# zepfu/llama-gguf-inference

Measured on AMD Instinct MI355X. Metric: decode tokens/sec + achieved HBM GB/s, Llama-3-8B Q4_K_M, 1->8 MI355X, higher is better.
Workload: dtype int8; 1 GPU; llama3-8b-q4km: 128-token prompt -> greedy decode on the 128->640 trajectory, 1521 timed tokens at positions 133..1653 (mean context of the trajectory), 1 replica per GPU; model=llama3-8b-q4km, parallelism=replicas x1 (RCCL weight fan-out), global_batch=1

## Files before the change

### llama-gguf-inference_amd/csrc/capi_hooks.cpp

```cpp
#include <hip/hip_runtime.h>

#include <algorithm>
#include <cstring>
#include <string>
#include <vector>

#include "../../include/llmi.h"
#include "capi_internal.h"

using namespace llmi;

extern "C" {

int32_t llmi_profile_kernels(struct llama_context* ctx, llama_token first, int32_t pos0, int32_t n_steps, double* us,
                             double* bytes, int32_t* launches) {
    API_TRY
    if (!ctx || n_steps <= 0 || !us || !bytes || !launches) { set_err("llmi_profile_kernels: bad arguments"); return -1; }
    Context& c = ctx->c;
    if (first < 0 || first >= c.m->hp.n_vocab || pos0 < 0 || pos0 >= c.n_ctx) {
        set_err("llmi_profile_kernels: token/position out of range");
        return -1;
    }
    (void)hipSetDevice(c.m->device);
    const int kv_bound = std::min(c.n_ctx, (pos0 / 256 + 1) * 256);
// ... 54 lines not shown
    if (!c.le_trace && hipMalloc(&c.le_trace, n * 8) != hipSuccess) { set_err("llmi_engine_trace: hipMalloc"); return -3; }
    (void)hipMemsetAsync(c.le_trace, 0, n * 8, c.stream);
    bool ok = launch_state_set(c.st, first, pos0, c.stream) == hipSuccess && step_enqueue(c, kv_bound, err);
    c.le_trace_layer = layer;
    ok = ok && launch_state_set(c.st, first, pos0, c.stream) == hipSuccess && step_enqueue(c, kv_bound, err);
    c.le_trace_layer = -1;
    if (!ok || hipMemcpyAsync(out, c.le_trace, n * 8, hipMemcpyDeviceToHost, c.stream) != hipSuccess ||
        hipStreamSynchronize(c.stream) != hipSuccess) {
        set_err("llmi_engine_trace: " + (err.empty() ? std::string("launch failed") : err));
        rc = -4;
    }
    if (launch_state_set(c.st, first, pos0, c.stream) != hipSuccess || hipStreamSynchronize(c.stream) != hipSuccess)
        if (rc == 0) { set_err("llmi_engine_trace: state reset failed"); rc = -4; }
    c.n_past = pos0;
    return rc == 0 ? cus : rc;
    API_CATCH(-5)
}

double llmi_le_stream_bench(const void* src, int64_t bytes, int32_t mode, int32_t iters, int32_t nt) {
    return le_stream_bench(src, (size_t)bytes, mode, iters, nt);
}

static thread_local int t_hook_numerics = 0;

int32_t llmi_test_option(const char* name, int32_t value) {
    if (!name) return -1;
    int* opt = nullptr;
    if (!strcmp(name, "numerics")) {
        const int old = t_hook_numerics;
        if (value >= 0 && value <= (NUMERICS_X86 | NUMERICS_FA)) t_hook_numerics = value;
        else if (value >= 0) { set_err("llmi_test_option: numerics must be 0..3"); return -1; }
        return old;
    }
    if (!strcmp(name, "pf_attn_simple")) opt = &g_pf_attn_simple;
    else if (!strcmp(name, "pf_fa_noalloc")) opt = &g_pf_fa_noalloc;
    else if (!strcmp(name, "pf_attn_fa")) opt = &g_pf_attn_fa;
    else if (!strcmp(name, "pf_gemm_ng")) opt = &g_pf_gemm_ng;
    else if (!strcmp(name, "pf_qkv_merge")) opt = &g_pf_qkv_merge;
    else if (!strcmp(name, "pf_xcd_map")) opt = &g_pf_xcd_map;
    else if (!strcmp(name, "pf_quant_bpc")) opt = &g_pf_quant_bpc;
    else if (!strcmp(name, "pf_quant_split_below")) opt = &g_pf_quant_split_below;
    else if (!strcmp(name, "pf_fa_cfg")) opt = &g_pf_fa_cfg;
    else if (!strcmp(name, "pf_max_kv")) opt = &g_pf_max_kv;
    else if (!strcmp(name, "xspin_limit")) opt = &g_xspin_limit;
    else if (!strcmp(name, "xtag_skew")) opt = &g_xtag_skew;
    else if (!strcmp(name, "engine")) opt = &g_le_on;
    else if (!strcmp(name, "le_spin")) opt = &g_le_spin;
    if (!opt) { set_err("llmi_test_option: unknown option"); return -1; }
    const int old = *opt;
    if (value >= 0) *opt = value;
    return old;
}

int32_t llmi_debug_tap(struct llama_context* ctx, int32_t which, float* out) {
    if (!ctx || !out) { set_err("llmi_debug_tap: bad arguments"); return -1; }
    Context& c = ctx->c;
    const HParams& hp = c.m->hp;
    (void)hipSetDevice(c.m->device);
    if (which == 7 || which == 8) {
        const size_t kvl = (size_t)hp.n_head_kv * c.n_ctx * hp.head_dim;
        const uint16_t* base = (which == 7 ? c.kc : c.vc) + (size_t)(hp.n_layer - 1) * kvl;
        hipError_t e = hipMemcpyAsync(out, base, kvl * 2, hipMemcpyDeviceToHost, c.stream);
        if (e == hipSuccess) e = hipStreamSynchronize(c.stream);
        if (e != hipSuccess) { set_err(hip_err(e)); return -2; }
        return 0;
    }
    if (which >= 11 && which <= 15) {
// ... 600 lines not shown
```

### llama-gguf-inference_amd/csrc/kernels.h

```cpp
#pragma once

#include <hip/hip_runtime.h>

#include <cstdint>
#include <string>

#include "common.h"

namespace llmi {

#ifndef LLMI_MV_THREADS
#define LLMI_MV_THREADS 256
#endif
constexpr int kMVThreads = LLMI_MV_THREADS;
constexpr int kMVWaves = kMVThreads / 64;
constexpr int kFusedAttnMaxKV = 8192;
constexpr size_t kSplitAttnMaxLds = 128 * 1024;
constexpr int kXAttnMaxKV = 1024;
constexpr int kDimAttnMaxKV = 1024;
constexpr int kRegAttnMaxKV = 512;
constexpr int kPfAttnMaxKV = 32768;
extern int g_pf_fa_noalloc, g_pf_gemm_ng, g_pf_qkv_merge, g_pf_xcd_map, g_pf_quant_bpc, g_pf_quant_split_below, g_pf_attn_simple, g_pf_attn_fa, g_pf_fa_cfg, g_pf_max_kv, g_xspin_limit, g_xtag_skew;
int pf_max_kv();
__host__ __device__ inline size_t attn_gran_off(int n_head, int n_ctx) {
    return ((size_t)n_head * n_ctx + (size_t)n_head * (n_ctx / 32 + 1) + 3) & ~(size_t)3;
}
constexpr int kLongTile = 256;
__host__ __device__ inline size_t attn_long_off(int n_head, int n_ctx) { return attn_gran_off(n_head, n_ctx) + 2 * (size_t)n_head * kXAttnMaxKV + 4; }
inline size_t attn_scratch_floats(int n_head, int n_ctx) {
    return attn_long_off(n_head, n_ctx) + 2 * (size_t)n_head * ((n_ctx + kLongTile - 1) / kLongTile) * 129;
}

enum Epi : int { EPI_STORE = 0, EPI_ADD = 1, EPI_QKV = 2, EPI_SWIGLU = 3, EPI_LOGITS = 4,
                 EPI_SWIGLU_UP = 5 };

struct Seg {
    const uint8_t* a = nullptr;
    const uint8_t* h = nullptr;
    const uint8_t* s = nullptr;
    const uint8_t* d = nullptr;
    int type = -1;
    int rows = 0;
    int row0 = 0;
    int rgs = 0;
    int x86 = 0;
};

struct MVArgs {
    Seg seg[3];
    int nseg = 0;
    int cols = 0;
    int npairs = 0;
    const float* x = nullptr;
    const float* nw = nullptr;
    const uint8_t* xq = nullptr;
    float eps = 0.f;
    float* y = nullptr;
    uint16_t* kc = nullptr;
    uint16_t* vc = nullptr;
    const float* rope = nullptr;
    StepState* st = nullptr;
    int head_dim = 0, n_rot = 0, n_ctx = 0, nq = 0, nk = 0;
    unsigned long long* argmax = nullptr;
    unsigned long long* trace = nullptr;
    int lr = 0;
    int rpt = 0;
    int ntasks = 0;
    int split_tasks = 0;
    int split_wgs = 0;
    int xfirst = 0;
    int fw = 0;
    int prio_alt = 0;
    int x_stride = 0, y_stride = 0;
    const int* tpos = nullptr;
    const int* tseq = nullptr;
    size_t kv_stride = 0;
    int num = 0;
};

constexpr int kLeOps = 4;
struct LeArgs {
    MVArgs op[kLeOps];
    int nops = 0;
    unsigned* cnt = nullptr;
    size_t cnt_stride = 0;
    unsigned* fault = nullptr;
    int spin_limit = 0;
    int kmin = 9;
    int npieces = 0, img_off0 = 0, img_off1 = 0, fold_off = 0, ring_off = 0, act = -1;
    int exp = 0;
    unsigned long long* trace = nullptr;
};
size_t le_counter_bytes(int n_layer);
size_t le_counter_stride(int n_layer);
hipError_t layer_engine_prepare(LeArgs& a);
hipError_t launch_layer_engine(const LeArgs& a, hipStream_t s);
double le_stream_bench(const void* src, size_t bytes, int mode, int iters, int nt);
bool le_wanted();
extern int g_le_on, g_le_spin;

// ... 70 lines not shown
    const float* rope = nullptr;
    int pos0 = 0, head_dim = 0, n_rot = 0, n_ctx = 0;
    int exp = 0;
};
struct PfAttn {
    const float* q = nullptr;
    float* out = nullptr;
    int ldq = 0;
    const uint16_t* kc = nullptr, *vc = nullptr;
    int n_ctx = 0, pos0 = 0, gqa = 1, max_kv = 0;
    float scale = 0.f;
    float* wsc = nullptr;
    size_t wsc_bytes = 0;
    int num = 0;
    int fa = 0;
};
size_t pf_fa_scratch_bytes(int n_head, int n_head_kv, int head_dim, int T, int n_ctx);
constexpr size_t kPfFaScratchCap = (size_t)1 << 30;
bool pf_gemm_ok(int type, int rows, int cols);
hipError_t launch_pf_embed(const Seg& w, int cols, int vocab, const int32_t* toks, float* X, int T, int32_t* hist,
                           int pos0, int n_ctx, hipStream_t s);
hipError_t launch_pf_quant(const float* x, int ldx, const float* nw, float eps, int cols, int act, int T, void* aq,
                           int16_t* abs, float* ad, void* abf, hipStream_t s, int x86 = 0);
hipError_t launch_pf_gemm(const PfGemm& g, int epi, hipStream_t s);
hipError_t launch_pf_attn(const PfAttn& a, int n_head, int head_dim, int T, hipStream_t s, int path = -1);

__host__ __device__ inline int act_kind(int t) { return t == T_Q8_0 ? 1 : 0; }
bool mv_geometry(MVArgs& a, int epi);
size_t mv_lds_bytes(int act, int cols);
template <int ACT, bool NORM, int T, int X86>
hipError_t mv_dispatch_epi(const MVArgs& a, int epi, dim3 grid, size_t lds, hipStream_t s);
template <bool NORM, int T, int T2, int X86>
hipError_t mv_qkv2_launch(const MVArgs& a, int split_tasks, dim3 grid, size_t lds, hipStream_t s);

hipError_t launch_matvec(const MVArgs& a, int epi, int max_blocks, hipStream_t stream);
int attn_path(int n_head, int n_head_kv, int kv_bound, int head_dim, int mode = -1);
int attn_d_slices(int n_head, int head_dim);
int battn_path(int g, int n_head, int head_dim, int kv_bound, int nt);
int battn_slices(int n_head, int head_dim, int kv_bound, int nt);
int attn_passes(int kv_bound, int cap);
struct LongGeo { int ntile, np, nscores; };
LongGeo attn_long_geo(int kv_bound);
void set_launch_events(hipEvent_t start, hipEvent_t stop);
void set_attn_mode(int mode);
constexpr int kFaMaxKV = 8192;
hipError_t launch_attention_fa(const AttnArgs& a, int n_head, int n_head_kv, int head_dim, int kv_bound, hipStream_t s);
hipError_t launch_battention_fa(const BAttnArgs& b, int nt, int n_head, int n_head_kv, int head_dim, int kv_bound,
                                hipStream_t s);
hipError_t launch_battention_x86(const BAttnArgs& b, int nt, int n_head, int n_head_kv, int head_dim, int kv_bound,
                                 hipStream_t s);
hipError_t launch_attention(const AttnArgs& a, int n_head, int n_head_kv, int head_dim, int kv_bound, hipStream_t stream,
                            int mode = -1);
hipError_t launch_embed(const EmbArgs& a, hipStream_t stream);
hipError_t launch_embed_row(const EmbArgs& a, const StepState* st, float* out, hipStream_t stream);
hipError_t launch_repack(int type, const void* raw, uint8_t* a, uint8_t* h, uint8_t* s, uint8_t* d, int64_t nblk, int64_t cols, int rgs,
                         int x86, hipStream_t stream);
hipError_t launch_attention_x86(const AttnArgs& a, int n_head, int n_head_kv, int head_dim, int kv_bound, hipStream_t s,
                                int mode = 0);
hipError_t launch_pf_attn_x86(const PfAttn& a, int n_head, int n_head_kv, int head_dim, int T, hipStream_t s);
int pf_attn_x86_max_kv(int n_head, int n_head_kv, int head_dim);
hipError_t launch_pf_attn_fa(const PfAttn& a, int n_head, int head_dim, int T, hipStream_t s);
hipError_t launch_quant_dump(const MVArgs& a, int act, void* out, hipStream_t stream);
hipError_t launch_stream_read(const void* p, size_t bytes, unsigned* out, int blocks, hipStream_t stream);
hipError_t launch_arena_hash(const void* p, size_t bytes, unsigned long long* out, hipStream_t stream);
hipError_t launch_state_set(StepState* st, int token_in, int pos_next, hipStream_t stream);
hipError_t launch_state_tick(StepState* st, hipStream_t stream);
// ... 3 lines not shown
```

### llama-gguf-inference_amd/csrc/kernels.hip

```cpp
#include "kernels.h"
#include "mv_device.h"
#include "launch_util.h"

#include <algorithm>
#include <cstdlib>

#include <hip/hip_runtime.h>

namespace llmi {

static thread_local hipEvent_t t_ev_start = nullptr, t_ev_stop = nullptr;
void set_launch_events(hipEvent_t start, hipEvent_t stop) {
    t_ev_start = start;
    t_ev_stop = stop;
}
hipEvent_t launch_event(bool stop) { return stop ? t_ev_stop : t_ev_start; }

size_t mv_lds_bytes(int act, int cols) { return fold_off(act, cols, kMVWaves) + (size_t)kMVWaves * kFoldFloats * 4; }

template <int ACT, int X86>
__global__ __launch_bounds__(kMVThreads) void k_quant_dump(MVArgs A, uint8_t* out) {
    extern __shared__ __attribute__((aligned(16))) uint8_t smem[];
    const Lds L = carve(smem, ACT, A.cols);
    if (A.nw) mv_prologue<ACT, true, X86>(A, L);
    else mv_prologue<ACT, false, X86>(A, L);
    __syncthreads();
    const int cols = A.cols;
    for (int e = threadIdx.x; e < cols; e += blockDim.x) {
        const uint8_t* rec = L.act + (size_t)(e >> 8) * kRec;
        const int t = e & 255;
        if (ACT == 0) {
            const int c = t >> 6, h = (t >> 5) & 1, l = X86 ? (t & 31) >> 2 : t & 7, i = X86 ? t & 3 : (t & 31) >> 3;
            out[(size_t)(e >> 8) * 292 + 4 + t] = rec[32 * (2 * c + (l >> 2)) + 16 * h + 4 * (l & 3) + i];
        } else {
            out[(size_t)(e >> 5) * 34 + 2 + (e & 31)] = rec[t];
        }
    }
    if (ACT == 0) {
// ... 198 lines not shown
    const int sp = split_row / a.rpt;
#define LLMI_QKV2(A_, B_)                                                                            \
    if (t1 == A_ && t2 == B_) return mv_qkv2_launch<NORM, A_, B_, X86>(a, sp, grid, lds, s);
    if constexpr (NORM) {
        LLMI_QKV2(T_Q4_K, T_Q6_K) LLMI_QKV2(T_Q4_K, T_Q5_K) LLMI_QKV2(T_Q5_K, T_Q6_K)
    }
#undef LLMI_QKV2
    return hipErrorNotSupported;
}

template <bool NORM, int X86>
static hipError_t mv_dispatch_type(const MVArgs& a, int epi, dim3 grid, size_t lds, hipStream_t s) {
    static const bool qkv2 = !getenv("LLMI_NO_QKV2");
    if (epi == EPI_QKV && qkv2) {
        const hipError_t e = mv_dispatch_qkv2<NORM, X86>(a, grid, lds, s);
        if (e != hipErrorNotSupported) return e;
    }
    int best = a.seg[0].type, best_rows = 0;
    for (int i = 0; i < a.nseg; ++i) {
        int rows = 0;
        for (int k = 0; k < a.nseg; ++k)
            if (a.seg[k].type == a.seg[i].type) rows += a.seg[k].rows;
        if (rows > best_rows) { best_rows = rows; best = a.seg[i].type; }
    }
    switch (best) {
        case T_Q4_K: return mv_dispatch_epi<0, NORM, T_Q4_K, X86>(a, epi, grid, lds, s);
        case T_Q5_K: return mv_dispatch_epi<0, NORM, T_Q5_K, X86>(a, epi, grid, lds, s);
        case T_Q6_K: return mv_dispatch_epi<0, NORM, T_Q6_K, X86>(a, epi, grid, lds, s);
        case T_Q8_0: return mv_dispatch_epi<1, NORM, T_Q8_0, X86>(a, epi, grid, lds, s);
        default: return hipErrorInvalidValue;
    }
}

bool mv_geometry(MVArgs& a, int epi) {
    if (a.nseg < 1 || a.cols < 256 || a.cols % 256) return false;
    const int U = a.cols >> 8, lmax = epi == EPI_QKV ? 32 : 64;
    static const int lr_cap = [] {
        const char* e = getenv("LLMI_MV_LR");
        return e ? atoi(e) : 64;
    }();
    int lr = (std::min(std::min(U, lmax), lr_cap) + 3) & ~3;
    lr = std::min(std::max(lr, 4), lmax);
    int R = 1;
    while (2 * R * lr <= 64) R *= 2;
    auto aligned = [&](int r) {
        for (int i = 1; i < a.nseg; ++i)
            if ((a.seg[i].row0 - a.seg[0].row0) % r) return false;
        return true;
    };
    if (epi != EPI_SWIGLU)
        while (R > 1 && !aligned(R)) R >>= 1;
    if (epi == EPI_QKV && R < 2) return false;
    int rows;
    if (epi == EPI_SWIGLU) {
        if (a.nseg != 2 || a.seg[0].rows != a.seg[1].rows) return false;
        rows = a.seg[0].rows;
    } else {
        rows = a.seg[a.nseg - 1].row0 + a.seg[a.nseg - 1].rows - a.seg[0].row0;
    }
    a.lr = lr;
    a.rpt = R;
    a.ntasks = (rows + R - 1) / R;
    return a.ntasks > 0;
}

static int mv_fw() {
    static const int v = [] {
        const char* e = getenv("LLMI_MV_FW");
        return e ? atoi(e) : 0;
    }();
    return v;
}

hipError_t launch_matvec(const MVArgs& a0, int epi, int max_blocks, hipStream_t s) {
    if (a0.nseg < 1 || a0.cols <= 0 || a0.cols % 256) return hipErrorInvalidValue;
    MVArgs a = a0;
    a.fw = mv_fw();
    if (!mv_geometry(a, epi)) return hipErrorInvalidValue;
    const int act = act_kind(a.seg[0].type);
    for (int i = 1; i < a.nseg; ++i)
        if (act_kind(a.seg[i].type) != act) return hipErrorInvalidValue;
    const size_t lds = mv_lds_bytes(act, a.cols);
    if (lds > 160 * 1024) return hipErrorInvalidValue;
    int blocks = (a.ntasks + kMVWaves - 1) / kMVWaves;
    if (blocks > max_blocks) blocks = max_blocks;
#if defined(LLMI_EXPERIMENTS)
    static const int exp_blocks = [] {
        const char* e = getenv("LLMI_MV_BLOCKS");
        return e ? atoi(e) : 0;
    }();
    if (exp_blocks > 0 && exp_blocks < blocks) blocks = exp_blocks;
#endif
    const dim3 grid(blocks);
    for (int i = 0; i < a.nseg; ++i)
        if ((a.seg[i].x86 != 0) != (a.num != 0)) return hipErrorInvalidValue;
    if (a.num) return a.nw ? mv_dispatch_type<true, 1>(a, epi, grid, lds, s) : mv_dispatch_type<false, 1>(a, epi, grid, lds, s);
    return a.nw ? mv_dispatch_type<true, 0>(a, epi, grid, lds, s) : mv_dispatch_type<false, 0>(a, epi, grid, lds, s);
}

hipError_t launch_quant_dump(const MVArgs& a, int act, void* out, hipStream_t s) {
    if (a.cols <= 0 || a.cols % 256) return hipErrorInvalidValue;
    const size_t lds = mv_lds_bytes(act, a.cols);
    if (a.num) {
        if (act == 0) hipLaunchKernelGGL((k_quant_dump<0, 1>), dim3(1), dim3(kMVThreads), lds, s, a, (uint8_t*)out);
        else hipLaunchKernelGGL((k_quant_dump<1, 1>), dim3(1), dim3(kMVThreads), lds, s, a, (uint8_t*)out);
    } else {
        if (act == 0) hipLaunchKernelGGL((k_quant_dump<0, 0>), dim3(1), dim3(kMVThreads), lds, s, a, (uint8_t*)out);
        else hipLaunchKernelGGL((k_quant_dump<1, 0>), dim3(1), dim3(kMVThreads), lds, s, a, (uint8_t*)out);
    }
    return hipGetLastError();
}
// ... 48 lines not shown
```

### llama-gguf-inference_amd/csrc/mv_device.h

```cpp
#pragma once

#include <hip/hip_runtime.h>

#include "kernels.h"
#include "../../include/llmi_math.h"

namespace llmi {

typedef unsigned int u32x4 __attribute__((ext_vector_type(4)));
typedef unsigned int u32x2 __attribute__((ext_vector_type(2)));
typedef int i32x4 __attribute__((ext_vector_type(4)));
typedef short short2_t __attribute__((ext_vector_type(2)));

#ifndef LLMI_NT
#define LLMI_NT 1
#endif
constexpr bool kNontemporalWeights = LLMI_NT != 0;

__device__ __forceinline__ float h2f(uint32_t h) {
    return (float)__builtin_bit_cast(_Float16, (uint16_t)(h & 0xffffu));
}
__device__ __forceinline__ uint16_t f2h(float f) {
    __asm__("" : "+v"(f));
    return __builtin_bit_cast(uint16_t, (_Float16)f);
// ... 1072 lines not shown
__device__ __forceinline__ void task_any(const MA& A, const Lds& L, float* F, const TaskGeo& g, int task, int r, int ul,
                                         int pos, unsigned long long& best) {
    const int S = EPI == EPI_SWIGLU ? 2 * g.nj : g.nj;
    float acc = 0.f, vg = 0.f;
    for (int s = 0; s < S; ++s) {
        const Sub b = sub_of<EPI>(A, g, task, s);
        const Seg sg = pick(A, b.si);
        const LaneUnit lu = lane_unit(g, b, sg, r, ul);
        const uint8_t* rec = L.act + (size_t)lu.u * kRec;
        float tm[9];
        if constexpr (X86) {
            if constexpr (ACT == 1) {
                unit_store_x86<T_Q8_0>(load_unit<T_Q8_0>(sg, lu.row, lu.u, g.U), rec, F, r, ul, g.lr, g.R, lu.valid);
            } else {
                switch (sg.type) {
                    case T_Q4_K: unit_store_x86<T_Q4_K>(load_unit<T_Q4_K>(sg, lu.row, lu.u, g.U), rec, F, r, ul, g.lr, g.R, lu.valid); break;
                    case T_Q5_K: unit_store_x86<T_Q5_K>(load_unit<T_Q5_K>(sg, lu.row, lu.u, g.U), rec, F, r, ul, g.lr, g.R, lu.valid); break;
                    default: unit_store_x86<T_Q6_K>(load_unit<T_Q6_K>(sg, lu.row, lu.u, g.U), rec, F, r, ul, g.lr, g.R, lu.valid); break;
                }
            }
        } else if constexpr (ACT == 1) {
            unit_terms<T_Q8_0>(load_unit<T_Q8_0>(sg, lu.row, lu.u, g.U), rec, tm);
        } else {
            switch (sg.type) {
                case T_Q4_K: unit_terms<T_Q4_K>(load_unit<T_Q4_K>(sg, lu.row, lu.u, g.U), rec, tm); break;
                case T_Q5_K: unit_terms<T_Q5_K>(load_unit<T_Q5_K>(sg, lu.row, lu.u, g.U), rec, tm); break;
                default: unit_terms<T_Q6_K>(load_unit<T_Q6_K>(sg, lu.row, lu.u, g.U), rec, tm); break;
            }
        }
        sub_finish<ACT, EPI, MA, X86>(A, F, g, s, b, sg, tm, lu, r, ul, acc, vg, pos, best);
    }
}

__device__ __forceinline__ float dequant_elem(const Seg& w, int row, int e, int cols) {
    const size_t U = (size_t)(cols >> 8), u = (size_t)(e >> 8), ru = (size_t)row * U + u;
    switch (w.type) {
        case T_F32: return ((const float*)w.a)[(size_t)row * cols + e];
        case T_F16: return h2f(((const uint16_t*)w.a)[(size_t)row * cols + e]);
        case T_Q4_K:
        case T_Q5_K:
        case T_Q6_K: {
            const int t = e & 255, c = t >> 6, hi = (t >> 5) & 1;
            const int l = w.x86 ? (t & 31) >> 2 : t & 7, i = w.x86 ? t & 3 : (t & 31) >> 3, k = l >> 2, m = l & 3;
            const uint8_t qb = w.a[piece_off(row, 2 * c + k, u, U, 8, w.rgs) + 4 * m + i];
            int q = hi ? (qb >> 4) : (qb & 0xF);
            if (w.type == T_Q6_K) {
                const uint8_t hb = w.h[piece_off(row, c, u, U, 4, w.rgs) + (2 * hi + k) * 4 + i];
                q |= (((hb >> (2 * m)) & 3) ^ 2) << 4;
                const float d = h2f(*(const uint16_t*)(w.d + ru * 2));
                const int sc = (int8_t)w.s[ru * 16 + (t >> 4)];
                return d * (float)sc * (float)(q - 32);
            }
            const uint32_t* s32 = (const uint32_t*)(w.s + ru * 16);
            int sc, mn;
            scale_min(2 * c + hi, s32[1], s32[2], s32[3], sc, mn);
            if (w.type == T_Q5_K) {
                const uint8_t hb = w.h[piece_off(row, c >> 1, u, U, 2, w.rgs) + 8 * (c & 1) + 4 * hi + i];
                q += ((hb >> l) & 1) << 4;
            }
            const float d = h2f(s32[0]), dmin = h2f(s32[0] >> 16);
            const float d1 = d * (float)sc, m1 = dmin * (float)mn;
            return d1 * (float)q - m1;
        }
        case T_Q8_0: {
            const int t = e & 255;
            const uint8_t qb = w.a[piece_off(row, t >> 4, u, U, 16, w.rgs) + (t & 15)];
// ... 20 lines not shown
```

### llama-gguf-inference_amd/csrc/mv_kernels.h

```cpp
#pragma once
#include "kernels.h"
#include "launch_util.h"
#include "mv_device.h"

#include <algorithm>
#include <cstdlib>
#include <map>
#include <mutex>
#include <tuple>

namespace llmi {

#ifndef LLMI_MV_PINGPONG
#define LLMI_MV_PINGPONG 1
#endif
#ifndef LLMI_Q6_MASKED
#define LLMI_Q6_MASKED 1
#endif
constexpr bool kQ6Masked = LLMI_Q6_MASKED != 0;
__host__ inline size_t mv_lds_total(int act, int cols, int nw, int t, int t2, int x86 = 0) {
    const int ff = fold_stride_cols(act, x86, cols);
    const size_t base = fold_off(act, cols, nw) + (size_t)nw * ff * 4;
    return base + ((kQ6Masked && !x86 && (t == T_Q6_K || t2 == T_Q6_K)) ? (size_t)(cols >> 8) * kQ6MaskRec : 0);
}

static int g_split_by_pairs = getenv("LLMI_SPLIT_BY_PAIRS") ? atoi(getenv("LLMI_SPLIT_BY_PAIRS")) : 0;


#if defined(LLMI_EXP_TRACE)
#define MV_STAMP(I, V)                                                                                    \
    if (A.trace && (threadIdx.x & 63) == 0)                                                               \
        A.trace[((size_t)blockIdx.x * (NT / 64) + (threadIdx.x >> 6)) * 16 + (I)] = (V);
#define MV_NOW __builtin_amdgcn_s_memrealtime()
#else
#define MV_STAMP(I, V)
#endif

template <int ACT, bool NORM, int EPI, int T, int NP, int NT = kMVThreads, int X86 = 0>
__device__ __forceinline__ unsigned long long mv_body(const MVArgs& A, const Lds& L, float* F, int t0, int G, int tbeg,
                                                      int tend) {
    int pos = 0;
    if constexpr (EPI == EPI_QKV) pos = A.st->pos;
    unsigned long long best = 0;
    const int lane = threadIdx.x & 63;
    const TaskGeo g = task_geo(A);
    const int S = EPI == EPI_SWIGLU ? 2 * g.nj : g.nj;
    const int r = lane / g.lr, ul = lane - r * g.lr;

    int task = t0;
    MV_STAMP(0, MV_NOW)
    [[maybe_unused]] int nsub_done = 0, nsub_alt = 0;
    ProRegs<NORM, NP> R;
    ImgRegs<2 * NP + 1> RI;
    const bool img = A.xq != nullptr;
    if (img) mv_img_issue<2 * NP + 1, NT>(A, RI);
    else mv_prologue_issue<NORM, NP, NT>(A, R);
    if ((tend - tbeg <= G && A.xfirst >= 0) || A.xfirst > 0) asm volatile("s_waitcnt vmcnt(0)" ::: "memory");
    const bool pipe = task < tend && task_is<EPI, T>(A, g, task);
    Sub b = sub_of<EPI>(A, g, task < tend ? task : tend - 1, 0);
    Seg sg = pick(A, b.si);
    LaneUnit lu = lane_unit(g, b, sg, r, ul);
    UnitW<T> cur = load_unit<T>(sg, pipe ? lu.row : 0u, pipe ? lu.u : 0u, g.U);
    if (img) mv_img_finish<2 * NP + 1, NT>(A, L, RI);
    else mv_prologue_finish<ACT, NORM, NP, NT, X86>(A, L, R);
    __syncthreads();
    [[maybe_unused]] uint8_t* q6m = nullptr;
    if constexpr (T == T_Q6_K && kQ6Masked && !X86) {
        q6m = (uint8_t*)L.act + fold_off(ACT, A.cols, NT / 64) + (size_t)(NT / 64) * kFoldFloats * 4;
        q6_masks_build<NT>(L, g.U, q6m);
        __syncthreads();
    }
    MV_STAMP(1, MV_NOW)

    if (pipe) {
        int s = 0;
        float acc = 0.f, vg = 0.f;
        bool first_sub = A.fw != 0;
        auto step = [&](UnitW<T>& cur, UnitW<T>& nxt) -> bool {
            int tn = task, sn = s + 1;
            Sub bn = b;
            Seg sgn = sg;
            bool has_next = true;
            if (sn == S) {
                sn = 0;
                tn = task + G;
                has_next = tn < tend && task_is<EPI, T>(A, g, tn);
            }
            if (has_next) {
                bn = sub_of<EPI>(A, g, tn, sn);
                sgn = pick(A, bn.si);
            }
            const LaneUnit lun = lane_unit(g, bn, sgn, r, ul);
            if (first_sub) {
                asm volatile("s_waitcnt vmcnt(0)" ::: "memory");
                first_sub = false;
            }
            nxt = load_unit<T>(sgn, has_next ? lun.row : 0u, has_next ? lun.u : 0u, g.U);
            float tm[9];
            if constexpr (X86)
                unit_store_x86<T>(cur, L.act + (size_t)lu.u * kRec, F, r, ul, g.lr, g.R, lu.valid);
            else if constexpr (T == T_Q6_K && kQ6Masked)
                unit_terms_q6m(cur, q6m + (size_t)lu.u * kQ6MaskRec, *(const float*)(L.act + (size_t)lu.u * kRec + kRecD), tm);
            else
                unit_terms<T>(cur, L.act + (size_t)lu.u * kRec, tm);
            sub_finish<ACT, EPI, MVArgs, X86>(A, F, g, s, b, sg, tm, lu, r, ul, acc, vg, pos, best);
#if defined(LLMI_EXP_TRACE)
            ++nsub_done;
            if (nsub_done == 1) { MV_STAMP(2, MV_NOW) }
            else if (nsub_done <= 9) { MV_STAMP(6 + nsub_done, MV_NOW) }
#endif
            task = tn;
            if (!has_next) return false;
            s = sn;
            b = bn;
            sg = sgn;
            lu = lun;
            return true;
        };
#if LLMI_MV_PINGPONG
        UnitW<T> other;
        for (;;) {
            if (!step(cur, other)) break;
            if (!step(other, cur)) break;
        }
#else
        for (;;) {
            UnitW<T> nxt;
            if (!step(cur, nxt)) break;
            cur = nxt;
        }
#endif
    }
    for (; task < tend; task += G) task_any<ACT, EPI, MVArgs, X86>(A, L, F, g, task, r, ul, pos, best);
    MV_STAMP(3, MV_NOW)
    MV_STAMP(5, ((unsigned long long)(__builtin_amdgcn_s_getreg(6164) & 15) << 32) | (unsigned)nsub_done)
    return best;
}

template <int ACT, bool NORM, int EPI, int T, int NP, int T2 = T, int NT = kMVThreads, int X86 = 0>
__global__ __launch_bounds__(NT) void k_matvec(MVArgs A) {
    constexpr int NW = NT / 64;
    extern __shared__ __attribute__((aligned(16))) uint8_t smem[];
    const Lds L = carve(smem, ACT, A.cols);
    const int wave = uniform((int)(threadIdx.x >> 6));
    const int lane = threadIdx.x & 63;
    float* F = (float*)(smem + fold_off(ACT, A.cols, NW)) + wave * fold_stride(ACT, X86, A.rpt, A.lr);
    unsigned long long best;
    if constexpr (T2 == T) {
        int t0 = blockIdx.x * NW + wave, G = gridDim.x * NW, tb = 0, te = A.ntasks;
        if (A.split_wgs > 0) {
            if ((int)blockIdx.x < A.split_wgs) {
                G = A.split_wgs * NW;
                te = A.split_tasks;
            } else {
                t0 = A.split_tasks + (blockIdx.x - A.split_wgs) * NW + wave;
                G = (gridDim.x - A.split_wgs) * NW;
                tb = A.split_tasks;
            }
        }
        best = mv_body<ACT, NORM, EPI, T, NP, NT, X86>(A, L, F, t0, G, tb, te);
    } else {
        if ((int)blockIdx.x < A.split_wgs)
            best = mv_body<ACT, NORM, EPI, T, NP, NT, X86>(A, L, F, blockIdx.x * NW + wave, A.split_wgs * NW, 0, A.split_tasks);
        else
            best = mv_body<ACT, NORM, EPI, T2, NP, NT, X86>(A, L, F, A.split_tasks + (blockIdx.x - A.split_wgs) * NW + wave,
                                                            (gridDim.x - A.split_wgs) * NW, A.split_tasks, A.ntasks);
    }
    if constexpr (EPI == EPI_LOGITS) {
        const int cur_pos = A.st->pos;
        unsigned long long* red = (unsigned long long*)L.red;
        best = wave_max_u64(best);
        __syncthreads();
        if (lane == 0) red[wave] = best;
        __syncthreads();
        if (threadIdx.x == 0) {
            unsigned long long b = red[0];
#pragma unroll
            for (int w = 1; w < NW; ++w) b = red[w] > b ? red[w] : b;
            if (b) atomicMax(&A.argmax[(cur_pos & 1) * kArgSlots + blockIdx.x % kArgSlots], b);
            if (blockIdx.x == 0) A.st->pos_next = cur_pos + 1;
        }
    }
}

template <typename K>
static dim3 resident_grid(K kernel, dim3 grid, size_t lds, int threads = kMVThreads) {
    static std::mutex mu;
    static std::map<std::tuple<const void*, size_t, int>, int> cache;
    int dev = 0;
    (void)hipGetDevice(&dev);
    const auto key = std::make_tuple((const void*)kernel, lds, dev * 4096 + threads);
    int cap = 0;
    {
        std::lock_guard<std::mutex> lk(mu);
        auto it = cache.find(key);
        if (it != cache.end()) {
            cap = it->second;
        } else {
// ... 149 lines not shown
    hipError_t e = hipSuccess;
    if (mv_try_wide<ACT, NORM, T, EPI, X86>(a, s, e)) return e;
    if (mv_try_narrow<ACT, NORM, T, EPI, X86>(a, s, e)) return e;
    switch (prologue_np(a.cols)) {
        case 1: return mv_launch<ACT, NORM, T, EPI, 1, X86>(a, grid, lds, s);
        case 2: return mv_launch<ACT, NORM, T, EPI, 2, X86>(a, grid, lds, s);
        default: return mv_launch<ACT, NORM, T, EPI, 4, X86>(a, grid, lds, s);
    }
}

template <int ACT, bool NORM, int T, int X86>
hipError_t mv_dispatch_epi(const MVArgs& a, int epi, dim3 grid, size_t lds, hipStream_t s) {
    switch (epi) {
        case EPI_STORE: return mv_launch_np<ACT, NORM, T, EPI_STORE, X86>(a, grid, lds, s);
        case EPI_ADD: return mv_launch_np<ACT, NORM, T, EPI_ADD, X86>(a, grid, lds, s);
        default: break;
    }
    if constexpr (NORM) {
        switch (epi) {
            case EPI_QKV: return mv_launch_np<ACT, NORM, T, EPI_QKV, X86>(a, grid, lds, s);
            case EPI_SWIGLU: return mv_launch_np<ACT, NORM, T, EPI_SWIGLU, X86>(a, grid, lds, s);
            case EPI_LOGITS: return mv_launch_np<ACT, NORM, T, EPI_LOGITS, X86>(a, grid, lds, s);
            default: break;
        }
    }
    return hipErrorInvalidValue;
}

template <bool NORM, int T, int T2, int X86>
hipError_t mv_qkv2_launch(const MVArgs& a, int split_tasks, dim3 grid, size_t lds, hipStream_t s) {
    return mv_launch2<0, NORM, T, T2, EPI_QKV, 1, X86>(a, split_tasks, grid, lds, s);
}

}
```

Before: 528.8 tokens/s.

## Split quantized super-blocks across lane pairs in decode matvec kernels

```diff
diff --git a/llama-gguf-inference_amd/csrc/capi_hooks.cpp b/llama-gguf-inference_amd/csrc/capi_hooks.cpp
--- a/llama-gguf-inference_amd/csrc/capi_hooks.cpp
+++ b/llama-gguf-inference_amd/csrc/capi_hooks.cpp
@@ -110,7 +110,14 @@
         else if (value >= 0) { set_err("llmi_test_option: numerics must be 0..3"); return -1; }
         return old;
     }
+    if (!strcmp(name, "mv_unit_split")) {
+        const int old = g_mv_unit_split;
+        if (value < -1 || value > 3) { set_err("llmi_test_option: mv_unit_split must be -1..3"); return -2; }
+        g_mv_unit_split = value;
+        return old;
+    }
     if (!strcmp(name, "pf_attn_simple")) opt = &g_pf_attn_simple;
+    else if (!strcmp(name, "mv_split_nt")) opt = &g_mv_split_nt;
     else if (!strcmp(name, "pf_fa_noalloc")) opt = &g_pf_fa_noalloc;
     else if (!strcmp(name, "pf_attn_fa")) opt = &g_pf_attn_fa;
     else if (!strcmp(name, "pf_gemm_ng")) opt = &g_pf_gemm_ng;
diff --git a/llama-gguf-inference_amd/csrc/kernels.h b/llama-gguf-inference_amd/csrc/kernels.h
--- a/llama-gguf-inference_amd/csrc/kernels.h
+++ b/llama-gguf-inference_amd/csrc/kernels.h
@@ -20,6 +20,7 @@
 constexpr int kDimAttnMaxKV = 1024;
 constexpr int kRegAttnMaxKV = 512;
 constexpr int kPfAttnMaxKV = 32768;
+extern int g_mv_unit_split, g_mv_split_nt;
 extern int g_pf_fa_noalloc, g_pf_gemm_ng, g_pf_qkv_merge, g_pf_xcd_map, g_pf_quant_bpc, g_pf_quant_split_below, g_pf_attn_simple, g_pf_attn_fa, g_pf_fa_cfg, g_pf_max_kv, g_xspin_limit, g_xtag_skew;
 int pf_max_kv();
 __host__ __device__ inline size_t attn_gran_off(int n_head, int n_ctx) {
@@ -66,6 +67,8 @@
     int lr = 0;
     int rpt = 0;
     int ntasks = 0;
+    int us = 1;
+    int us2 = 0, lr2 = 0, rpt2 = 0, t2beg = 0, t2end = 0;
     int split_tasks = 0;
     int split_wgs = 0;
     int xfirst = 0;
@@ -202,6 +205,10 @@
 hipError_t mv_dispatch_epi(const MVArgs& a, int epi, dim3 grid, size_t lds, hipStream_t s);
 template <bool NORM, int T, int T2, int X86>
 hipError_t mv_qkv2_launch(const MVArgs& a, int split_tasks, dim3 grid, size_t lds, hipStream_t s);
+template <bool NORM, int T, int X86>
+hipError_t mv_split_launch(const MVArgs& a, int epi, int nt, hipStream_t s);
+template <int X86, int US>
+hipError_t mv_split_qkv2_launch(const MVArgs& a, int nt, hipStream_t s);
 
 hipError_t launch_matvec(const MVArgs& a, int epi, int max_blocks, hipStream_t stream);
 int attn_path(int n_head, int n_head_kv, int kv_bound, int head_dim, int mode = -1);
diff --git a/llama-gguf-inference_amd/csrc/kernels.hip b/llama-gguf-inference_amd/csrc/kernels.hip
--- a/llama-gguf-inference_amd/csrc/kernels.hip
+++ b/llama-gguf-inference_amd/csrc/kernels.hip
@@ -4,6 +4,7 @@
 
 #include <algorithm>
 #include <cstdlib>
+#include <cstring>
 
 #include <hip/hip_runtime.h>
 
@@ -268,16 +269,16 @@
     }
 }
 
-bool mv_geometry(MVArgs& a, int epi) {
-    if (a.nseg < 1 || a.cols < 256 || a.cols % 256) return false;
-    const int U = a.cols >> 8, lmax = epi == EPI_QKV ? 32 : 64;
+static void mv_geo_lanes(const MVArgs& a, int epi, int us, int& lr, int& R) {
+    const int U = a.cols >> 8, lmax = (epi == EPI_QKV ? 32 : 64) / us;
     static const int lr_cap = [] {
         const char* e = getenv("LLMI_MV_LR");
         return e ? atoi(e) : 64;
     }();
-    int lr = (std::min(std::min(U, lmax), lr_cap) + 3) & ~3;
-    lr = std::min(std::max(lr, 4), lmax);
-    int R = 1;
+    int lu = (std::min(std::min(U, lmax), lr_cap) + 3) & ~3;
+    lu = std::min(std::max(lu, 4), lmax);
+    lr = lu * us;
+    R = 1;
     while (2 * R * lr <= 64) R *= 2;
     auto aligned = [&](int r) {
         for (int i = 1; i < a.nseg; ++i)
@@ -286,7 +287,17 @@
     };
     if (epi != EPI_SWIGLU)
         while (R > 1 && !aligned(R)) R >>= 1;
+}
+bool mv_geometry(MVArgs& a, int epi) {
+    if (a.nseg < 1 || a.cols < 256 || a.cols % 256 || (a.us != 1 && a.us != 2)) return false;
+    int lr, R;
+    mv_geo_lanes(a, epi, a.us, lr, R);
     if (epi == EPI_QKV && R < 2) return false;
+    if (a.us2) {
+        if (a.us2 != 1 && a.us2 != 2) return false;
+        mv_geo_lanes(a, epi, a.us2, a.lr2, a.rpt2);
+        if (epi == EPI_QKV && a.rpt2 < 2) return false;
+    }
     int rows;
     if (epi == EPI_SWIGLU) {
         if (a.nseg != 2 || a.seg[0].rows != a.seg[1].rows) return false;
@@ -308,11 +319,87 @@
     return v;
 }
 
+int g_mv_unit_split = -1;
+int g_mv_split_nt = 0;
+static int mv_split_mode() {
+    static const int env = [] {
+        const char* e = getenv("LLMI_MV_SPLIT");
+        return e && strcmp(e, "auto") ? atoi(e) : -1;
+    }();
+    const int m = g_mv_unit_split >= 0 ? g_mv_unit_split : env;
+    return m < 0 || m > 3 ? 3 : m;
+}
+static int mv_split_nt() {
+    static const int env = [] {
+        const char* e = getenv("LLMI_MV_SPLIT_NT");
+        return e ? atoi(e) : 0;
+    }();
+    const int v = g_mv_split_nt ? g_mv_split_nt : env;
+    return v == 256 || v == 512 ? v : 256;
+}
+static int mv_split_plan(MVArgs& a, int epi, int max_blocks) {
+    static const bool qkv2 = !getenv("LLMI_NO_QKV2");
+    const int mode = mv_split_mode();
+    if (mode == 0 || !(epi == EPI_STORE || epi == EPI_ADD || epi == EPI_QKV)) return 0;
+    if (epi == EPI_QKV && !a.nw) return 0;
+    int t1 = a.seg[0].type, t2 = -1;
+    for (int i = 1; i < a.nseg; ++i) {
+        if (a.seg[i].type == (t2 < 0 ? t1 : t2)) continue;
+        if (t2 >= 0) return 0;
+        t2 = a.seg[i].type;
+    }
+    const int waves = max_blocks * kMVWaves;
+    MVArgs g = a;
+    if (t2 < 0) {
+        if ((t1 != T_Q4_K && t1 != T_Q6_K) || mode == 2) return 0;
+        if (!mv_geometry(g, epi)) return 0;
+        if (mode == 3 && g.ntasks > waves) return 0;
+        g.us = 2;
+        if (!mv_geometry(g, epi)) return 0;
+        a.us = 2;
+        return 1;
+    }
+    if (epi != EPI_QKV || !qkv2 || t1 != T_Q4_K || t2 != T_Q6_K || a.cols > 16 * kMVThreads) return 0;
+    a.us = mode == 1 ? 2 : 1;
+    a.us2 = 2;
+    return 2;
+}
+
 hipError_t launch_matvec(const MVArgs& a0, int epi, int max_blocks, hipStream_t s) {
     if (a0.nseg < 1 || a0.cols <= 0 || a0.cols % 256) return hipErrorInvalidValue;
     MVArgs a = a0;
     a.fw = mv_fw();
+    a.us = 1;
+    a.us2 = 0;
+    const int split = act_kind(a.seg[0].type) == 0 ? mv_split_plan(a, epi, max_blocks) : 0;
     if (!mv_geometry(a, epi)) return hipErrorInvalidValue;
+    if (split) {
+        for (int i = 0; i < a.nseg; ++i)
+            if (act_kind(a.seg[i].type) != 0 || (a.seg[i].x86 != 0) != (a.num != 0)) return hipErrorInvalidValue;
+        const int nt = mv_split_nt();
+        if (split == 1) {
+            const int t = a.seg[0].type;
+#define LLMI_SPLIT1(N_, T_, X_) return mv_split_launch<N_, T_, X_>(a, epi, nt, s)
+            if (a.nw) {
+                if (t == T_Q4_K) { if (a.num) LLMI_SPLIT1(true, T_Q4_K, 1); else LLMI_SPLIT1(true, T_Q4_K, 0); }
+                else { if (a.num) LLMI_SPLIT1(true, T_Q6_K, 1); else LLMI_SPLIT1(true, T_Q6_K, 0); }
+            } else {
+                if (t == T_Q4_K) { if (a.num) LLMI_SPLIT1(false, T_Q4_K, 1); else LLMI_SPLIT1(false, T_Q4_K, 0); }
+                else { if (a.num) LLMI_SPLIT1(false, T_Q6_K, 1); else LLMI_SPLIT1(false, T_Q6_K, 0); }
+            }
+#undef LLMI_SPLIT1
+        }
+        int split_row = 0;
+        for (int i = a.nseg - 1; i >= 1; --i)
+            if (a.seg[i].type == T_Q6_K) split_row = a.seg[i].row0 - a.seg[0].row0;
+        const int rows = a.seg[a.nseg - 1].row0 + a.seg[a.nseg - 1].rows - a.seg[0].row0;
+        if (split_row <= 0 || split_row % a.rpt || split_row % a.rpt2) return hipErrorInvalidValue;
+        a.split_tasks = split_row / a.rpt;
+        a.t2beg = split_row / a.rpt2;
+        a.t2end = (rows + a.rpt2 - 1) / a.rpt2;
+        if (a.us == 2) return a.num ? mv_split_qkv2_launch<1, 2>(a, nt, s) : mv_split_qkv2_launch<0, 2>(a, nt, s);
+        return a.num ? mv_split_qkv2_launch<1, 1>(a, nt, s) : mv_split_qkv2_launch<0, 1>(a, nt, s);
+    }
     const int act = act_kind(a.seg[0].type);
     for (int i = 1; i < a.nseg; ++i)
         if (act_kind(a.seg[i].type) != act) return hipErrorInvalidValue;
diff --git a/llama-gguf-inference_amd/csrc/mv_device.h b/llama-gguf-inference_amd/csrc/mv_device.h
--- a/llama-gguf-inference_amd/csrc/mv_device.h
+++ b/llama-gguf-inference_amd/csrc/mv_device.h
@@ -1128,6 +1128,193 @@
     }
 }
 
+__host__ __device__ inline TaskGeo task_geo_split(const MVArgs& A, int lanes, int R) {
+    TaskGeo g;
+    g.lr = lanes >> 1;
+    g.R = R;
+    g.U = A.cols >> 8;
+    g.nj = (g.U + g.lr - 1) / g.lr;
+    return g;
+}
+template <int T>
+struct HalfW {
+    u32x4 q[4];
+    u32x4 s;
+    u32x4 h[2];
+    uint32_t d;
+};
+template <int T>
+__device__ __forceinline__ HalfW<T> load_half(const Seg& sg, uint32_t row, uint32_t u, uint32_t U, uint32_t half) {
+    static_assert(T == T_Q4_K || T == T_Q6_K, "split units: Q4_K and Q6_K");
+    HalfW<T> w;
+    const uint32_t P = (U * 16) << sg.rgs, ru = row * U + u;
+    const uint32_t oa = piece_off(row, 0, u, U, 8, sg.rgs) + 4 * half * P;
+#pragma unroll
+    for (int p = 0; p < 4; ++p) w.q[p] = ldw(sg.a + oa + (uint32_t)p * P);
+    if constexpr (T == T_Q4_K) {
+        w.s = ldw(sg.s + ru * 16);
+        w.d = 0;
+    } else {
+        const u32x2 s2 = ldw8(sg.s + ru * 16 + 8 * half);
+        w.s = u32x4{s2.x, s2.y, 0u, 0u};
+        const uint32_t oh = piece_off(row, 0, u, U, 4, sg.rgs) + 2 * half * P;
+        w.h[0] = ldw(sg.h + oh);
+        w.h[1] = ldw(sg.h + oh + P);
+        w.d = *(const uint16_t*)(sg.d + ru * 2);
+    }
+    return w;
+}
+__device__ __forceinline__ void join_halves(int (&t)[8]) {
+#pragma unroll
+    for (int l = 0; l < 8; ++l) t[l] += xor_partner_i<1>(t[l]);
+}
+__device__ __forceinline__ void half_ints_q4(const HalfW<T_Q4_K>& w, const uint8_t* rec, uint32_t half, int (&t)[8],
+                                             int (&pr)[2]) {
+    u32x2 sc, mn;
+    scales_mins(w.s.y, w.s.z, w.s.w, sc, mn);
+    const uint32_t sw = half ? sc.y : sc.x, mw = half ? mn.y : mn.x;
+    const uint8_t* a = rec + 128 * half;
+#pragma unroll
+    for (int l = 0; l < 8; ++l) t[l] = 0;
+#pragma unroll
+    for (int p = 0; p < 4; ++p) {
+        const int c = p >> 1, k = p & 1;
+        const int slo = (int)((sw >> (16 * c)) & 0xffu), shi = (int)((sw >> (16 * c + 8)) & 0xffu);
+        const i32x4 alo = *(const i32x4*)(a + 32 * p), ahi = *(const i32x4*)(a + 32 * p + 16);
+#pragma unroll
+        for (int m = 0; m < 4; ++m) {
+            const int l = 4 * k + m;
+            const uint32_t l4 = w.q[p][m] & M4, h4 = (w.q[p][m] >> 4) & M4;
+            t[l] = __mul24(slo, dot4z(l4, alo[m])) + t[l];
+            t[l] = __mul24(shi, dot4z(h4, ahi[m])) + t[l];
+        }
+    }
+    const i32x4 bs = *(const i32x4*)(rec + kRecBs + 16 * half);
+    pr[0] = 0;
+    pr[1] = 0;
+#pragma unroll
+    for (int j = 0; j < 4; ++j) {
+        const uint32_t sel = 0x0c000c00u | (uint32_t)j * 0x00010001u;
+        const uint32_t mm = __builtin_amdgcn_perm(0u, mw, sel);
+        const int bp = bs[j];
+        pr[j >> 1] = __builtin_amdgcn_sdot2(__builtin_bit_cast(short2_t, bp), __builtin_bit_cast(short2_t, mm), pr[j >> 1], false);
+    }
+}
+template <bool MASKED>
+__device__ __forceinline__ void half_ints_q6(const HalfW<T_Q6_K>& w, const uint8_t* a, int (&t)[8]) {
+#pragma unroll
+    for (int l = 0; l < 8; ++l) t[l] = 0;
+#pragma unroll
+    for (int p = 0; p < 4; ++p) {
+        const int c = p >> 1, k = p & 1;
+        const uint32_t s4 = c ? w.s.y : w.s.x;
+        const int c0 = (int)(int8_t)(s4 & 0xff), c1 = (int)(int8_t)((s4 >> 8) & 0xff),
+                  c2 = (int)(int8_t)((s4 >> 16) & 0xff), c3 = (int)(int8_t)(s4 >> 24);
+        i32x4 a0, a1, a2, a3;
+        if constexpr (MASKED) {
+            a0 = *(const i32x4*)(a + 64 * p), a1 = *(const i32x4*)(a + 64 * p + 16);
+            a2 = *(const i32x4*)(a + 64 * p + 32), a3 = *(const i32x4*)(a + 64 * p + 48);
+        } else {
+            const i32x4 alo = *(const i32x4*)(a + 32 * p), ahi = *(const i32x4*)(a + 32 * p + 16);
+            a0 = alo & 0xffff, a1 = alo & (int)0xffff0000u, a2 = ahi & 0xffff, a3 = ahi & (int)0xffff0000u;
+        }
+        const uint32_t hl = w.h[c][k], hh = w.h[c][2 + k];
+#pragma unroll
+        for (int m = 0; m < 4; ++m) {
+            const uint32_t q = w.q[p][m];
+            const uint32_t wl = (q & M4) | q6_hi_bytes((hl >> (2 * m)) & M2);
+            const uint32_t wh = ((q >> 4) & M4) | q6_hi_bytes((hh >> (2 * m)) & M2);
+            int v = t[4 * k + m];
+            v = __mul24(c0, dot4z(wl, a0[m])) + v;
+            v = __mul24(c1, dot4z(wl, a1[m])) + v;
+            v = __mul24(c2, dot4z(wh, a2[m])) + v;
+            v = __mul24(c3, dot4z(wh, a3[m])) + v;
+            t[4 * k + m] = v;
+        }
+    }
+}
+__device__ __forceinline__ void half_ints_q6_x86(const HalfW<T_Q6_K>& w, const uint8_t* a, int (&t)[8]) {
+#pragma unroll
+    for (int l = 0; l < 8; ++l) t[l] = 0;
+#pragma unroll
+    for (int p = 0; p < 4; ++p) {
+        const int c = p >> 1, k = p & 1;
+        const uint32_t s4 = c ? w.s.y : w.s.x;
+        const int clo = (int)(int8_t)((s4 >> (8 * k)) & 0xff), chi = (int)(int8_t)((s4 >> (8 * (2 + k))) & 0xff);
+        const i32x4 alo = *(const i32x4*)(a + 32 * p), ahi = *(const i32x4*)(a + 32 * p + 16);
+        const uint32_t hl = w.h[c][k], hh = w.h[c][2 + k];
+#pragma unroll
+        for (int m = 0; m < 4; ++m) {
+            const uint32_t q = w.q[p][m];
+            const uint32_t wl = (q & M4) | q6_hi_bytes((hl >> (2 * m)) & M2);
+            const uint32_t wh = ((q >> 4) & M4) | q6_hi_bytes((hh >> (2 * m)) & M2);
+            int v = t[4 * k + m];
+            v = __mul24(clo, dot4z(wl, alo[m])) + v;
+            v = __mul24(chi, dot4z(wh, ahi[m])) + v;
+            t[4 * k + m] = v;
+        }
+    }
+}
+template <int T, bool MASKED>
+__device__ __forceinline__ void half_terms(const HalfW<T>& w, const uint8_t* rec, const uint8_t* q6m, uint32_t half,
+                                           float (&tm)[9]) {
+    int t[8];
+    const float da = *(const float*)(rec + kRecD);
+    if constexpr (T == T_Q4_K) {
+        int pr[2];
+        half_ints_q4(w, rec, half, t, pr);
+        join_halves(t);
+        int sumi = pr[0] + pr[1];
+        sumi += xor_partner_i<1>(sumi);
+        const float d = h2f(w.s.x) * da, dm = h2f(w.s.x >> 16) * da;
+#pragma unroll
+        for (int l = 0; l < 8; ++l) tm[l] = d * (float)t[l];
+        tm[8] = -(dm * (float)sumi);
+    } else {
+        if constexpr (MASKED) half_ints_q6<true>(w, q6m + 256 * half, t);
+        else half_ints_q6<false>(w, rec + 128 * half, t);
+        join_halves(t);
+        const float d = h2f(w.d) * da;
+#pragma unroll
+        for (int l = 0; l < 8; ++l) tm[l] = d * (float)t[l];
+        tm[8] = 0.f;
+    }
+}
+template <int T>
+__device__ __forceinline__ void half_store_x86(const HalfW<T>& w, const uint8_t* rec, uint32_t half, float* F, int r,
+                                               int ul, int lr, bool store) {
+    int t[8];
+    float d, dm = 0.f;
+    float ms[4] = {0.f, 0.f, 0.f, 0.f};
+    const float da = *(const float*)(rec + kRecD);
+    if constexpr (T == T_Q4_K) {
+        int pr[2];
+        half_ints_q4(w, rec, half, t, pr);
+        join_halves(t);
+        const int q0 = xor_partner_i<1>(pr[0]), q1 = xor_partner_i<1>(pr[1]);
+        ms[0] = (float)pr[0];
+        ms[1] = (float)pr[1];
+        ms[2] = (float)q0;
+        ms[3] = (float)q1;
+        d = da * h2f(w.s.x);
+        dm = -da * h2f(w.s.x >> 16);
+    } else {
+        half_ints_q6_x86(w, rec + 128 * half, t);
+        join_halves(t);
+        d = da * h2f(w.d);
+    }
+    if (store) {
+        float* S = F + (size_t)r * 12 * lr + ul;
+#pragma unroll
+        for (int l = 0; l < 8; ++l) S[l * lr] = (float)t[l];
+#pragma unroll
+        for (int k = 0; k < 4; ++k) S[(8 + k) * lr] = ms[k];
+        float* D = F + kX86KD + (size_t)r * 2 * lr + ul;
+        D[0] = d;
+        D[lr] = dm;
+    }
+}
+
 __device__ __forceinline__ float dequant_elem(const Seg& w, int row, int e, int cols) {
     const size_t U = (size_t)(cols >> 8), u = (size_t)(e >> 8), ru = (size_t)row * U + u;
     switch (w.type) {
diff --git a/llama-gguf-inference_amd/csrc/mv_kernels.h b/llama-gguf-inference_amd/csrc/mv_kernels.h
--- a/llama-gguf-inference_amd/csrc/mv_kernels.h
+++ b/llama-gguf-inference_amd/csrc/mv_kernels.h
@@ -8,6 +8,7 @@
 #include <map>
 #include <mutex>
 #include <tuple>
+#include <type_traits>
 
 namespace llmi {
 
@@ -36,16 +37,22 @@
 #define MV_STAMP(I, V)
 #endif
 
-template <int ACT, bool NORM, int EPI, int T, int NP, int NT = kMVThreads, int X86 = 0>
-__device__ __forceinline__ unsigned long long mv_body(const MVArgs& A, const Lds& L, float* F, int t0, int G, int tbeg,
-                                                      int tend) {
+template <int ACT, bool NORM, int EPI, int T, int NP, int NT = kMVThreads, int X86 = 0, int US = 1>
+__device__ __forceinline__ unsigned long long mv_body(const MVArgs& A, const Lds& L, float* F, const TaskGeo& g, int t0,
+                                                      int G, int tbeg, int tend) {
+    using W = std::conditional_t<US == 2, HalfW<US == 2 ? T : T_Q4_K>, UnitW<T>>;
     int pos = 0;
     if constexpr (EPI == EPI_QKV) pos = A.st->pos;
     unsigned long long best = 0;
     const int lane = threadIdx.x & 63;
-    const TaskGeo g = task_geo(A);
     const int S = EPI == EPI_SWIGLU ? 2 * g.nj : g.nj;
-    const int r = lane / g.lr, ul = lane - r * g.lr;
+    const int slot = US == 2 ? lane >> 1 : lane;
+    [[maybe_unused]] const uint32_t half = lane & 1;
+    const int r = slot / g.lr, ul = slot - r * g.lr;
+    const auto load = [&](const Seg& s, uint32_t row, uint32_t u) {
+        if constexpr (US == 2) return load_half<T>(s, row, u, g.U, half);
+        else return load_unit<T>(s, row, u, g.U);
+    };
 
     int task = t0;
     MV_STAMP(0, MV_NOW)
@@ -60,7 +67,7 @@
     Sub b = sub_of<EPI>(A, g, task < tend ? task : tend - 1, 0);
     Seg sg = pick(A, b.si);
     LaneUnit lu = lane_unit(g, b, sg, r, ul);
-    UnitW<T> cur = load_unit<T>(sg, pipe ? lu.row : 0u, pipe ? lu.u : 0u, g.U);
+    W cur = load(sg, pipe ? lu.row : 0u, pipe ? lu.u : 0u);
     if (img) mv_img_finish<2 * NP + 1, NT>(A, L, RI);
     else mv_prologue_finish<ACT, NORM, NP, NT, X86>(A, L, R);
     __syncthreads();
@@ -76,7 +83,7 @@
         int s = 0;
         float acc = 0.f, vg = 0.f;
         bool first_sub = A.fw != 0;
-        auto step = [&](UnitW<T>& cur, UnitW<T>& nxt) -> bool {
+        auto step = [&](W& cur, W& nxt) -> bool {
             int tn = task, sn = s + 1;
             Sub bn = b;
             Seg sgn = sg;
@@ -95,8 +102,21 @@
                 asm volatile("s_waitcnt vmcnt(0)" ::: "memory");
                 first_sub = false;
             }
-            nxt = load_unit<T>(sgn, has_next ? lun.row : 0u, has_next ? lun.u : 0u, g.U);
+            nxt = load(sgn, has_next ? lun.row : 0u, has_next ? lun.u : 0u);
             float tm[9];
+            if constexpr (US == 2) {
+                const uint8_t* rec = L.act + (size_t)lu.u * kRec;
+                LaneUnit le = lu;
+                le.valid = lu.valid && half == 0;
+                if constexpr (X86) {
+                    half_store_x86<T>(cur, rec, half, F, r, ul, g.lr, le.valid);
+                } else {
+                    const uint8_t* mrec = nullptr;
+                    if constexpr (T == T_Q6_K && kQ6Masked) mrec = q6m + (size_t)lu.u * kQ6MaskRec;
+                    half_terms<T, kQ6Masked>(cur, rec, mrec, half, tm);
+                }
+                sub_finish<ACT, EPI, MVArgs, X86>(A, F, g, s, b, sg, tm, le, r, ul, acc, vg, pos, best);
+            } else {
             if constexpr (X86)
                 unit_store_x86<T>(cur, L.act + (size_t)lu.u * kRec, F, r, ul, g.lr, g.R, lu.valid);
             else if constexpr (T == T_Q6_K && kQ6Masked)
@@ -104,6 +124,7 @@
             else
                 unit_terms<T>(cur, L.act + (size_t)lu.u * kRec, tm);
             sub_finish<ACT, EPI, MVArgs, X86>(A, F, g, s, b, sg, tm, lu, r, ul, acc, vg, pos, best);
+            }
 #if defined(LLMI_EXP_TRACE)
             ++nsub_done;
             if (nsub_done == 1) { MV_STAMP(2, MV_NOW) }
@@ -118,20 +139,21 @@
             return true;
         };
 #if LLMI_MV_PINGPONG
-        UnitW<T> other;
+        W other;
         for (;;) {
             if (!step(cur, other)) break;
             if (!step(other, cur)) break;
         }
 #else
         for (;;) {
-            UnitW<T> nxt;
+            W nxt;
             if (!step(cur, nxt)) break;
             cur = nxt;
         }
 #endif
     }
-    for (; task < tend; task += G) task_any<ACT, EPI, MVArgs, X86>(A, L, F, g, task, r, ul, pos, best);
+    if constexpr (US == 1)
+        for (; task < tend; task += G) task_any<ACT, EPI, MVArgs, X86>(A, L, F, g, task, r, ul, pos, best);
     MV_STAMP(3, MV_NOW)
     MV_STAMP(5, ((unsigned long long)(__builtin_amdgcn_s_getreg(6164) & 15) << 32) | (unsigned)nsub_done)
     return best;
@@ -158,12 +180,12 @@
                 tb = A.split_tasks;
             }
         }
-        best = mv_body<ACT, NORM, EPI, T, NP, NT, X86>(A, L, F, t0, G, tb, te);
+        best = mv_body<ACT, NORM, EPI, T, NP, NT, X86>(A, L, F, task_geo(A), t0, G, tb, te);
     } else {
         if ((int)blockIdx.x < A.split_wgs)
-            best = mv_body<ACT, NORM, EPI, T, NP, NT, X86>(A, L, F, blockIdx.x * NW + wave, A.split_wgs * NW, 0, A.split_tasks);
+            best = mv_body<ACT, NORM, EPI, T, NP, NT, X86>(A, L, F, task_geo(A), blockIdx.x * NW + wave, A.split_wgs * NW, 0, A.split_tasks);
         else
-            best = mv_body<ACT, NORM, EPI, T2, NP, NT, X86>(A, L, F, A.split_tasks + (blockIdx.x - A.split_wgs) * NW + wave,
+            best = mv_body<ACT, NORM, EPI, T2, NP, NT, X86>(A, L, F, task_geo(A), A.split_tasks + (blockIdx.x - A.split_wgs) * NW + wave,
                                                             (gridDim.x - A.split_wgs) * NW, A.split_tasks, A.ntasks);
     }
     if constexpr (EPI == EPI_LOGITS) {
@@ -379,4 +401,85 @@
     return mv_launch2<0, NORM, T, T2, EPI_QKV, 1, X86>(a, split_tasks, grid, lds, s);
 }
 
-}
+template <bool NORM, int EPI, int T, int T2, int NT, int X86, int US, int US2>
+__global__ __launch_bounds__(NT) void k_matvec_split(MVArgs A) {
+    constexpr int NW = NT / 64;
+    extern __shared__ __attribute__((aligned(16))) uint8_t smem[];
+    const Lds L = carve(smem, 0, A.cols);
+    const int wave = uniform((int)(threadIdx.x >> 6));
+    float* F = (float*)(smem + fold_off(0, A.cols, NW)) + wave * fold_stride(0, X86, 1, 4);
+    if constexpr (T2 == T) {
+        static_assert(US == 2 && US2 == 2, "single-type split launches split every unit");
+        mv_body<0, NORM, EPI, T, 1, NT, X86, 2>(A, L, F, task_geo_split(A, A.lr, A.rpt), blockIdx.x * NW + wave,
+                                                 gridDim.x * NW, 0, A.ntasks);
+    } else {
+        if ((int)blockIdx.x < A.split_wgs) {
+            const TaskGeo g = US == 2 ? task_geo_split(A, A.lr, A.rpt) : task_geo(A);
+            mv_body<0, NORM, EPI, T, 1, NT, X86, US>(A, L, F, g, blockIdx.x * NW + wave, A.split_wgs * NW, 0, A.split_tasks);
+        } else {
+            const int bi = (int)blockIdx.x - A.split_wgs, nb2 = (int)gridDim.x - A.split_wgs;
+            TaskGeo g = task_geo_split(A, A.lr2, A.rpt2);
+            if constexpr (US2 == 1) {
+                g.lr = A.lr2;
+                g.nj = (g.U + g.lr - 1) / g.lr;
+            }
+            mv_body<0, NORM, EPI, T2, 1, NT, X86, US2>(A, L, F, g, A.t2beg + bi * NW + wave, nb2 * NW, A.t2beg, A.t2end);
+        }
+    }
+}
+
+template <bool NORM, int EPI, int T, int NT, int X86>
+static hipError_t mv_split_launch_nt(const MVArgs& a, hipStream_t s) {
+    constexpr int NW = NT / 64;
+    const size_t lds = mv_lds_total(0, a.cols, NW, T, T, X86);
+    if (lds > 160 * 1024) return hipErrorInvalidValue;
+    auto k = k_matvec_split<NORM, EPI, T, T, NT, X86, 2, 2>;
+    const dim3 g = resident_grid(k, dim3((a.ntasks + NW - 1) / NW), lds, NT);
+    launch_k(k, g, dim3(NT), lds, s, true, true, a);
+    return hipGetLastError();
+}
+template <bool NORM, int T, int X86>
+hipError_t mv_split_launch(const MVArgs& a, int epi, int nt, hipStream_t s) {
+    if (a.us != 2 || (nt != 256 && nt != 512)) return hipErrorInvalidValue;
+    for (int i = 0; i < a.nseg; ++i)
+        if (a.seg[i].type != T) return hipErrorInvalidValue;
+#define LLMI_SPLIT_NT(E_) (nt == 512 ? mv_split_launch_nt<NORM, E_, T, 512, X86>(a, s) : mv_split_launch_nt<NORM, E_, T, 256, X86>(a, s))
+    if (epi == EPI_STORE) return LLMI_SPLIT_NT(EPI_STORE);
+    if (epi == EPI_ADD) return LLMI_SPLIT_NT(EPI_ADD);
+    if constexpr (NORM)
+        if (epi == EPI_QKV) return LLMI_SPLIT_NT(EPI_QKV);
+#undef LLMI_SPLIT_NT
+    return hipErrorInvalidValue;
+}
+
+static inline int split_groups_nw(int wgs, int nw, int p1, int p2, double b1, double b2) {
+    int best = 1;
+    double best_cost = 1e300;
+    for (int w1 = 1; w1 < wgs; ++w1) {
+        const int n1 = w1 * nw, n2 = (wgs - w1) * nw;
+        const double c = std::max((double)((p1 + n1 - 1) / n1) * b1, (double)((p2 + n2 - 1) / n2) * b2);
+        if (c < best_cost) { best_cost = c; best = w1; }
+    }
+    return best;
+}
+template <int NT, int X86, int US>
+static hipError_t mv_split_qkv2_launch_nt(const MVArgs& a0, hipStream_t s) {
+    constexpr int NW = NT / 64;
+    const size_t lds = mv_lds_total(0, a0.cols, NW, T_Q4_K, T_Q6_K, X86);
+    if (lds > 160 * 1024) return hipErrorInvalidValue;
+    auto k = k_matvec_split<true, EPI_QKV, T_Q4_K, T_Q6_K, NT, X86, US, 2>;
+    MVArgs a = a0;
+    const int p1 = a.split_tasks, p2 = a.t2end - a.t2beg;
+    const dim3 g = resident_grid(k, dim3((p1 + NW - 1) / NW + (p2 + NW - 1) / NW), lds, NT);
+    if (g.x < 2) return hipErrorInvalidValue;
+    a.split_wgs = split_groups_nw((int)g.x, NW, p1, p2, US == 2 ? 1.0 : 2.0, 2.4);
+    launch_k(k, g, dim3(NT), lds, s, true, true, a);
+    return hipGetLastError();
+}
+template <int X86, int US>
+hipError_t mv_split_qkv2_launch(const MVArgs& a, int nt, hipStream_t s) {
+    if (a.us != US || a.us2 != 2 || a.nseg < 2 || a.cols > 16 * 256 || (nt != 256 && nt != 512)) return hipErrorInvalidValue;
+    return nt == 512 ? mv_split_qkv2_launch_nt<512, X86, US>(a, s) : mv_split_qkv2_launch_nt<256, X86, US>(a, s);
+}
+
+}
diff --git a/llama-gguf-inference_amd/csrc/mv_split.hip b/llama-gguf-inference_amd/csrc/mv_split.hip
--- /dev/null
+++ b/llama-gguf-inference_amd/csrc/mv_split.hip
@@ -0,0 +1,12 @@
+#ifndef LLMI_MV_X86
+#define LLMI_MV_X86 0
+#endif
+#include "mv_kernels.h"
+namespace llmi {
+template hipError_t mv_split_launch<true, T_Q4_K, LLMI_MV_X86>(const MVArgs&, int, int, hipStream_t);
+template hipError_t mv_split_launch<false, T_Q4_K, LLMI_MV_X86>(const MVArgs&, int, int, hipStream_t);
+template hipError_t mv_split_launch<true, T_Q6_K, LLMI_MV_X86>(const MVArgs&, int, int, hipStream_t);
+template hipError_t mv_split_launch<false, T_Q6_K, LLMI_MV_X86>(const MVArgs&, int, int, hipStream_t);
+template hipError_t mv_split_qkv2_launch<LLMI_MV_X86, 1>(const MVArgs&, int, hipStream_t);
+template hipError_t mv_split_qkv2_launch<LLMI_MV_X86, 2>(const MVArgs&, int, hipStream_t);
+}
diff --git a/llama-gguf-inference_amd/csrc/mv_split_x86.hip b/llama-gguf-inference_amd/csrc/mv_split_x86.hip
--- /dev/null
+++ b/llama-gguf-inference_amd/csrc/mv_split_x86.hip
@@ -0,0 +1,2 @@
+#define LLMI_MV_X86 1
+#include "mv_split.hip"
```

After: 537.4 tokens/s (median of 6 runs). +1.6%, better.
